# avik-pal/RegNeuralDE.jl

Hardware: AMD Instinct MI355X
Metric: training-step samples/sec + mean NFE, MNIST Neural ODE bs=512 (higher is better)
Workload: dtype f32; 1 GPU; MNIST NODE regularized (error_est), Tsit5 reltol=abstol=1.4e-8, batch 512 per GPU, 1xMI355X per rank; step = loss fwd + reverse pass through the solver + InvDecay/Momentum update; the weights train during the timed steps (mean_nfe drifts with --steps: value_fixed_weights of --full is the stationary companion); global_batch=512, parallelism=single

## Files before the change

regneuralde.jl_amd/csrc/rnde.hip:

```cpp
#include "rnde_node.h"

static thread_local std::string g_create_err;
extern "C" const char* rnde_version(void) { return "rnde 0.1.0 (gfx950)"; }
extern "C" const char* rnde_last_error(const rnde_node* h) { return h ? h->err.c_str() : g_create_err.c_str(); }

extern "C" int32_t rnde_param_count(const rnde_node_config* c) {
    int n = 0;
    for (int l = 0; l < c->n_layers; ++l) n += (c->dims[l] + (c->time_dep ? 1 : 0)) * c->dims[l + 1] + c->dims[l + 1];
    return n;
}

StepParams make_params(rnde_node* h, const float* x, int B, float t0, float t1, int tape) {
    StepParams P{};
    P.x = x;
    P.f0 = h->f0; P.h0 = h->h0; P.u1 = h->u1; P.f1 = h->f1; P.h1 = h->h1;
    P.arena = h->arena; P.rec_stride = h->rec_stride;
    P.ctl = h->ctl; P.ctl_final = h->ctl_final; P.meta = h->meta; P.initrec = h->initrec;
    P.errpart = h->errpart; P.initpart = h->initpart; P.dbg_out = nullptr;
    P.D = h->D; P.H = h->H; P.B = B; P.Bn = h->couple ? h->couple_batch : B;
    P.Bpad = ((B + 15) / 16) * 16;
    P.nwg = h->engine == 2 ? h->sR * (P.Bpad / 16) : (h->engine == 3 ? (h->mw ? P.Bpad / 16 : (P.Bpad / 16 + kCW - 1) / kCW) : P.Bpad / h->BT);
    P.reltol = h->cfg.reltol; P.abstol = h->cfg.abstol; P.t0 = t0; P.t1 = t1;
    P.tape = tape; P.max_attempts = h->cfg.max_attempts;
    P.forced = 0; P.forced_t = 0; P.forced_dt = 0;
// ... 513 lines not shown
    int n = 0;
    auto add = [&](void* dst, long long total, int kind, int which, int kdim, const float* src = nullptr) { J.j[n++] = PackJob{dst, src, total, kind, which, kdim, 0}; };
    add(h->spwB, (long long)h->sMT * h->sK2b * 64, 0, 0, h->sK2b);
    add(h->spwD, (long long)h->sHT * h->sMT * 64, 0, 1, h->sMT);
    add(h->spwBt, (long long)h->sMT * h->sKHb * 64, 0, 2, h->sKHb);
    add(h->spwDt, (long long)h->sHT * h->sMT * 64, 0, 3, h->sMT);
    auto add_copy = [&](float* dst, const float* src, long long floats) {
        const bool v4 = floats % 4 == 0 && ((uintptr_t)dst % 16 == 0) && ((uintptr_t)(src ? src : p_dev) % 16 == 0);
        add(dst, v4 ? floats / 4 : floats, v4 ? 3 : 2, 0, 0, src);
    };
    add_copy(h->pcopy, nullptr, (long long)h->P);
    if (x_src) add_copy(h->xcopy, x_src, x_floats);
    long long most = 0;
    for (int i = 0; i < n; ++i) most = std::max(most, J.j[i].total);
    const int grid = (int)std::min<long long>((most + 255) / 256, 256);
    hipLaunchKernelGGL(rnde_pack_all_kernel, dim3(grid, n), dim3(256), 0, s, p_dev, J, h->D, h->H);
    HIPCHK(h, hipGetLastError());
    h->rev_packed = true;
    return x3_pack(h, p_dev, true, s);
}
hipError_t slab_prepare(rnde_node* h, int Bpad, hipStream_t s) {
    if (h->tslab_Bpad == Bpad) return hipSuccess;
    h->tslab_Bpad = Bpad;
    return hipMemsetAsync(h->tslab, 0xFF, h->tslab_bytes, s);
}
static bool stage_two_tile(const rnde_node* h, const StageParams& Q) {
    const bool fix = Q.WT == 7 && Q.HT == 7 && Q.K2b == 7 && Q.MT == 49 && Q.R == 7 && h->D == 784 && h->H == 100 && !h->stage_generic;
    return h->persist == 1 && fix && Q.C % 2 == 0 && h->persist2 != 0 && (Q.C >= kPersist2MinTiles || h->persist2 >= 1);
}
static bool stage_epart_reduce(const rnde_node* h, const StageParams& Q) {
    return stage_two_tile(h, Q) && Q.F.nwg >= 896 && !getenv("RNDE_NO_EPART_REDUCE");
}
static hipError_t stage_attempt(rnde_node* h, const StageParams& Q, int n, hipStream_t s) {
// ... 231 lines not shown
            h->mw_solve = -1; h->mw_clean = 0; ++h->persist_fallbacks;
            hipMemsetAsync(h->mw_abort, 0, 8, s);
            return RNDE_INTERNAL_RETRY;
        }
        if (!h->h_ctl->done && h->h_ctl->n_att >= n_limit && n_limit < cap) { h->predicted = cap; return RNDE_INTERNAL_RETRY; }
        h->pending_bwd = false;
        ++h->one_launch_solves;
        solved = true;
    }
    if (h->engine == 2 && h->persist == 1 && h->stage_solve && h->sxch && SQ.C <= 32 && n_saveat == 0 && h->n_replay == 0 && !h->couple &&
        SQ.WT == 7 && SQ.HT == 7 && SQ.K2b == 7 && SQ.MT == 49 && SQ.R == 7 && h->D == 784 && h->H == 100 && !h->stage_generic) {
        PersistSync Y{h->tslab, h->pabort, h->pxcc, h->persist_spins};
        HIPCHK(h, slab_prepare(h, SQ.Bpad16, s));
        if (++h->s_epoch >= 500000u) { h->s_epoch = 1; HIPCHK(h, hipMemsetAsync(h->sxch, 0, (size_t)(cap + 1) * 3 * 256 * 8, s)); }
        const int x3 = h->x3_fwd ? 1 : 0;
        SolveSync Z{h->sxch, h->s_epoch, cap, h->x3B, h->x3D};
#ifdef RNDE_DIAG
        StageParams SD = SQ;
        if (getenv("RNDE_DIAG_SOLVE")) {
            if (h->diag_buf) hipFree(h->diag_buf);
            hipMalloc((void**)&h->diag_buf, 16384);
            hipMemsetAsync(h->diag_buf, 0, 16384, s);
            SD.F.dbg_out = h->diag_buf;
        }
        HIPCHK(h, rnde_launch_stage_solve(&SD, &Y, &Z, h->act2, x3, s));
#else
        HIPCHK(h, rnde_launch_stage_solve(&SQ, &Y, &Z, h->act2, x3, s));
#endif
        if (h->timing) { HIPCHK(h, hipEventRecord(h->tev[1], s)); h->tev_fwd = true; }
        hipLaunchKernelGGL(rnde_stage_finish_kernel, dim3(256), dim3(256), 0, s, SQ, -1, u_out_dev); HIPCHK(h, hipGetLastError());
        const int cnt = std::min(cap, std::max(64, 2 * h->predicted));
        HIPCHK(h, hipMemcpyAsync(h->h_mbox, h->mbox, h->mbox_meta_off + (size_t)cnt * sizeof(StepMeta), hipMemcpyDeviceToHost, s));
        if (h->after_solve) {
            HIPCHK(h, hipEventRecord(h->ev_host, s));
            const rnde_status hs = h->after_solve(s);
            if (hs != RNDE_OK) return hs;
            HIPCHK(h, hipEventSynchronize(h->ev_host));
        } else HIPCHK(h, hipStreamSynchronize(s));
#ifdef RNDE_DIAG
        if (getenv("RNDE_DIAG_SOLVE") && h->diag_buf) {
            static unsigned long long hst[1024];
            hipMemcpy(hst, h->diag_buf, 8192, hipMemcpyDeviceToHost);
            int na = 0; while (na < 119 && hst[(na + 1) * 8]) ++na;
            double acc[7] = {0}; int cnt = 0;
            for (int a = 2; a + 1 < na; ++a, ++cnt) {
// ... 431 lines not shown
```

regneuralde.jl_amd/csrc/rnde_bwd.h:

```cpp
#pragma once
#include "rnde_fwd.h"

namespace rnde {

struct BState {
    double tb_pre, dtb_pre, qoldb, t1b, t0b, pad[3];
};
struct IBState {
    double tb, t1b, t0b, dt0b, d1b, d2b, coef_w, pad;
};
struct EvalDesc {
    const float* Z;
    const float* X;
    float t;
    int pad;
};

struct BwdParams {
    StepParams F;
    float* U; float* K1; float* UB1;
    float* zi2; float* zi1;
    const float* svb_att;
    BState* bstate;
    IBState* ibstate;
// ... 79 lines not shown
static __global__ __launch_bounds__(64) void rnde_bpart_reduce_kernel(const BwdParams Q, int m, double* __restrict__ out) {
    const int lane = threadIdx.x;
    const float* part = Q.bpart + (size_t)(m & 1) * Q.bpart_n * 4;
    double S = 0, tau = 0, ctau = 0;
    for (int base = 0; base < Q.bpart_n; base += 256) {
        f32x4 e[4];
#pragma unroll
        for (int q = 0; q < 4; ++q) e[q] = *(const f32x4*)(part + 4 * (size_t)(base + lane + 64 * q));
#pragma unroll
        for (int q = 0; q < 4; ++q) if (base + lane + 64 * q < Q.bpart_n) { S += (double)e[q][0]; tau += (double)e[q][1]; ctau += (double)e[q][2]; }
    }
    S = wave_sum_d(S); tau = wave_sum_d(tau); ctau = wave_sum_d(ctau);
    if (lane == 0) { double* o = out + 4 * (m & 1); o[0] = S; o[1] = tau; o[2] = ctau; o[3] = 0; }
}

static __global__ __launch_bounds__(64) void rnde_bfin_kernel(const BwdParams Q) {
    const int lane = threadIdx.x;
    const IBState ib = Q.ibstate[1];
    double tau0 = 0;
    for (int i = lane; i < Q.F.nwg; i += 64) tau0 += (double)Q.ipart[((size_t)Q.F.nwg + i) * 4];
    tau0 = wave_sum_d(tau0);
    if (lane == 0) {
        const double sc = Q.tspan_scale != 0.f ? (double)Q.tspan_scale : 1.0;
        Q.tspan_out[0] = (float)(sc * (ib.t0b + tau0 + ib.tb));
        Q.tspan_out[1] = (float)(sc * ib.t1b);
    }
}

typedef float f32x16 __attribute__((ext_vector_type(16)));
__device__ __forceinline__ f32x4 mfma16(float a, float b, f32x4 c);

template <int MB, int NB>
__global__ __launch_bounds__(64) void rnde_wgrad_kernel(const EvalDesc* __restrict__ evals, int n_evals, int per_chunk,
                                                        int M, int Nx, int Bpad, float* __restrict__ slab) {
    const int lane = threadIdx.x, l31 = lane & 31, kk = lane >> 5;
    const int mtiles = (M + 31) / 32, ntiles = (Nx + 2 + 31) / 32;
    const int mblocks = (mtiles + MB - 1) / MB;
    const int mb = blockIdx.x % mblocks, nb = blockIdx.x / mblocks;
    const int chunk = blockIdx.y;
    const int e0 = chunk * per_chunk, e1 = min(n_evals, e0 + per_chunk);
    f32x16 acc[MB][NB];
#pragma unroll
// ... 274 lines not shown
        int c = c0;
        for (; c + 8 <= c1; c += 8) {
            float v[8];
#pragma unroll
            for (int j = 0; j < 8; ++j) v[j] = __builtin_nontemporal_load(slab + (size_t)(c + j) * len + i);
#pragma unroll
            for (int j = 0; j < 8; ++j) s += v[j];
        }
        for (; c < c1; ++c) s += __builtin_nontemporal_load(slab + (size_t)c * len + i);
        o[i] = s;
    }
}

struct ReduceJob { const float* slab; float* out; long long len; int n_chunks, per_group; };
struct ReducePair { ReduceJob j[2]; };
static __global__ void rnde_wgrad_reduce_pair(const ReducePair R) {
    const ReduceJob J = R.j[blockIdx.z];
    const int c0 = blockIdx.y * J.per_group, c1 = min(J.n_chunks, c0 + J.per_group);
    if (c0 >= c1) return;
    float* o = J.out + (size_t)blockIdx.y * J.len;
    for (long long i = blockIdx.x * (long long)blockDim.x + threadIdx.x; i < J.len; i += (long long)gridDim.x * blockDim.x) {
        float s = 0.f;
        int c = c0;
        for (; c + 8 <= c1; c += 8) {
            float v[8];
#pragma unroll
            for (int j = 0; j < 8; ++j) v[j] = __builtin_nontemporal_load(J.slab + (size_t)(c + j) * J.len + i);
#pragma unroll
            for (int j = 0; j < 8; ++j) s += v[j];
        }
        for (; c < c1; ++c) s += __builtin_nontemporal_load(J.slab + (size_t)c * J.len + i);
        o[i] = s;
    }
}

}
```

regneuralde.jl_amd/csrc/rnde_node.h:

```cpp
#pragma once
#include "../../include/rnde.h"
#include "rnde_fwd.h"
#include "rnde_bwd.h"
#include "rnde_stage.h"
#include "rnde_bstage.h"
#include "rnde_stage_persist2.h"
#include "rnde_bstage_persist.h"
#include "rnde_solve_sync.h"
#include "rnde_binit_stage.h"
#include "rnde_head.h"
#include "rnde_chain.h"
#include "rk_tables.h"
#include "rnde_bchain.h"
#include "rnde_chainmw.h"
#include "rnde_bchainmw.h"

#include <chrono>
#include <algorithm>
#include <atomic>
#include <cmath>
#include <cstdlib>
#include <cstdio>
#include <cstring>
#include <functional>
// ... 70 lines not shown
    int n_saveval = 0;
    int timing = 0; hipEvent_t tev[5] = {nullptr, nullptr, nullptr, nullptr, nullptr}; bool tev_fwd = false, tev_bwd = false;
    std::string err;
};

#define HIPCHK(h, call)                                                                              \
    do {                                                                                             \
        hipError_t e__ = (call);                                                                     \
        if (e__ != hipSuccess) {                                                                     \
            (h)->err = std::string(#call) + ": " + hipGetErrorString(e__);                           \
            return RNDE_ERR_HIP;                                                                     \
        }                                                                                            \
    } while (0)

static const rnde_status RNDE_INTERNAL_RETRY = static_cast<rnde_status>(100);
StepParams make_params(rnde_node* h, const float* x, int B, float t0, float t1, int tape);
MwParams make_mw_params(rnde_node* h, const StepParams& P);
ChainParams make_chain_params(rnde_node* h, const StepParams& P);
rnde_status couple_sum(rnde_node* h, float* partials, long long count, hipStream_t s);
hipError_t stage_pack(rnde_node* h, const float* p, f32x4* dst, int which, int MTrows, int Kb, hipStream_t st);
rnde_status stage_pack_all(rnde_node* h, const float* p_dev, hipStream_t s, const float* x_src = nullptr, long long x_floats = 0);
hipError_t slab_prepare(rnde_node* h, int Bpad, hipStream_t s);
void persist_check_enqueue(rnde_node* h, int grid, hipStream_t s);
bool persist_check_result(rnde_node* h, int C, int R, hipStream_t s);
bool bsweep_failed(rnde_node* h, hipStream_t s);
rnde_status forward_impl(rnde_node* h, const float* x_dev, const float* p_dev, int32_t B, float t0, float t1,
                         float* u_out_dev, const float* saveat_host, int32_t n_saveat, float* sv_out_dev,
                         int64_t* nfe_out, float* saveval_host, int32_t* n_saveval_out, int32_t keep_tape, void* stream);
```

regneuralde.jl_amd/csrc/rnde_reverse.hip:

```cpp
#include "rnde_node.h"
#include "rnde_wgradx.h"

static rnde_status chain_bwd_run(rnde_node* h, const float* u_bar_dev, const float* saveval_bar_host, float* x_bar_dev,
                                 float* p_bar_dev, float* tspan_bar_host, hipStream_t s, bool sync = true, float* tspan_bar_dev = nullptr);
static rnde_status bwd_run(rnde_node* h, const float* u_bar_dev, const float* saveval_bar_host, float* x_bar_dev,
                           float* p_bar_dev, float* tspan_bar_host, hipStream_t s, bool sync = true, float* tspan_bar_dev = nullptr);


extern "C" rnde_status rnde_node_backward_async(rnde_node* h, const float* u_bar_dev, const float* saveval_bar_host, float* x_bar_dev,
                                                float* p_bar_dev, float* tspan_bar_dev, void* stream) {
    if (!h) return RNDE_ERR_BAD_ARG;
    if (!h->have_tape) { h->err = "no recorded forward"; return RNDE_ERR_NO_TAPE; }
    if (h->engine == 3) return chain_bwd_run(h, u_bar_dev, saveval_bar_host, x_bar_dev, p_bar_dev, nullptr, (hipStream_t)stream, false, tspan_bar_dev);
    return bwd_run(h, u_bar_dev, saveval_bar_host, x_bar_dev, p_bar_dev, nullptr, (hipStream_t)stream, false, tspan_bar_dev);
}

extern "C" rnde_status rnde_node_backward(rnde_node* h, const float* u_bar_dev, const float* saveval_bar_host,
                                          float* x_bar_dev, float* p_bar_dev, float* tspan_bar_host, void* stream) {
    if (!h) return RNDE_ERR_BAD_ARG;
    if (!h->have_tape) { h->err = "no recorded forward"; return RNDE_ERR_NO_TAPE; }
    if (h->engine == 3) return chain_bwd_run(h, u_bar_dev, saveval_bar_host, x_bar_dev, p_bar_dev, tspan_bar_host, (hipStream_t)stream);
    return bwd_run(h, u_bar_dev, saveval_bar_host, x_bar_dev, p_bar_dev, tspan_bar_host, (hipStream_t)stream);
}
extern "C" rnde_status rnde_node_backward_host(rnde_node* h, const float* u_bar, const float* saveval_bar, float* x_bar,
// ... 138 lines not shown
        if ((size_t)(*chunk_cursor + sc) * (size_t)len > h->bw.slab_floats) { h->err = "weight-gradient slab overflow"; return RNDE_ERR_BAD_ARG; }
        if (tall) hipLaunchKernelGGL((rnde_wgrad2_kernel<true>), dim3(pblocks, sc), dim3(256), 0, s, ev, n_evals, steps_per_chunk, M, Nx, Bpad, dst);
        else hipLaunchKernelGGL((rnde_wgrad2_kernel<false>), dim3(pblocks, sc), dim3(256), 0, s, ev, n_evals, steps_per_chunk, M, Nx, Bpad, dst);
        HIPCHK(h, hipGetLastError());
        *chunk_cursor += sc;
        return RNDE_OK;
    } else {
        if ((size_t)(*chunk_cursor + chunks) * (size_t)len > h->bw.slab_floats) { h->err = "weight-gradient slab overflow"; return RNDE_ERR_BAD_ARG; }
        if (tall) hipLaunchKernelGGL((rnde_wgrad_kernel<2, 4>), dim3(blocks, chunks), dim3(64), 0, s, ev, n_evals, per_chunk, M, Nx, Bpad, dst);
        else hipLaunchKernelGGL((rnde_wgrad_kernel<4, 2>), dim3(blocks, chunks), dim3(64), 0, s, ev, n_evals, per_chunk, M, Nx, Bpad, dst);
    }
    HIPCHK(h, hipGetLastError());
    *chunk_cursor += chunks;
    return RNDE_OK;
}
static rnde_status launch_wgrad_reduce(rnde_node* h, const float* slab, int chunks, int M, int Nx, float* out, hipStream_t s) {
    const long long len = (long long)M * (Nx + 2);
    const int grid = (int)std::min<long long>((len + 255) / 256, 2048);
    if (chunks <= 16) {
        hipLaunchKernelGGL(rnde_wgrad_reduce, dim3(grid, 1), dim3(256), 0, s, slab, chunks, chunks, len, out);
    } else {
        const int per_group = (chunks + 15) / 16, groups = (chunks + per_group - 1) / per_group;
        hipLaunchKernelGGL(rnde_wgrad_reduce, dim3(grid, groups), dim3(256), 0, s, slab, chunks, per_group, len, h->bw.slab_r);
        hipLaunchKernelGGL(rnde_wgrad_reduce, dim3(grid, 1), dim3(256), 0, s, (const float*)h->bw.slab_r, groups, groups, len, out);
    }
    HIPCHK(h, hipGetLastError());
    return RNDE_OK;
}

static rnde_status bwd_run(rnde_node* h, const float* u_bar_dev, const float* saveval_bar_host, float* x_bar_dev,
                           float* p_bar_dev, float* tspan_bar_host, hipStream_t s, bool sync, float* tspan_bar_dev) {
    HIPCHK(h, hipSetDevice(h->cfg.device));
    rnde_status st = bwd_prepare(h);
    if (st != RNDE_OK) return st;
    BwdBuffers& b = h->bw;
    int n_att = h->n_att;
    const float svb_scale = h->couple ? (float)h->couple_world : 1.f;
    for (int i = 0; i < n_att; ++i)
        b.h_svb[i] = (saveval_bar_host && h->sv_index[i] >= 0) ? svb_scale * saveval_bar_host[h->sv_index[i]] : 0.f;
// ... 23 lines not shown
    for (int n = 0; n < n_att; ++n) {
        const StepMeta& m = h->h_meta[n];
        const float* R = h->arena + (long long)m.rec * h->rec_stride;
        for (int sidx = 2; sidx <= 7; ++sidx) {
            const float ts = m.t + tsC(sidx - 1) * m.dt;
            h_ev2[ne] = EvalDesc{R + L.k(sidx), R + L.h(sidx), ts, 0};
            h_ev1[ne] = EvalDesc{R + L.z1(sidx), sidx < 7 ? R + L.g(sidx) : R + L.unew(), ts, 0};
            ++ne;
        }
    }
    HIPCHK(h, hipMemcpyAsync(b.ev1, b.h_ev1, 2 * (size_t)ne * sizeof(EvalDesc) + (size_t)n_att * 4, hipMemcpyHostToDevice, s));
    float* slab1 = b.slab;
    float* slab2w = b.slab + b.slab_floats;
    int cur1 = 0, cur2 = 0, evi = 0;
    const int per_chunk = std::max(1, (ne + 239) / 240);
    const int side_pct = h->wgrad_side_pct;
    const int sweep_cus = 8 * h->sR * ((Q.F.Bpad / 16 + 7) / 8);
    const bool side = h->engine == 2 && h->persist == 1 && side_pct > 0 && n_att >= 8 && sweep_cus <= 224 &&
                      wgrad3_ok(h->H, h->D) && wgrad3_ok(h->D, h->H);
    const int side_att = side ? std::min(n_att, n_att * side_pct / 100) : 0;
    const int group = std::max(4, (side_att + 5) / 6);
    bool used_side = false;
    auto wgrad_group = [&](int lo, int hi, bool on_side) -> rnde_status {
        if (hi <= lo) return RNDE_OK;
        hipStream_t ws = s;
        if (on_side) {
            hipEvent_t ev = h->wevents[evi++ % 64];
            HIPCHK(h, hipEventRecord(ev, s));
            HIPCHK(h, hipStreamWaitEvent(h->wstream, ev, 0));
            ws = h->wstream; used_side = true;
        }
        rnde_status r = launch_wgrad_part(h, d_ev1 + lo, hi - lo, per_chunk, h->H, h->D, h->B, slab1, &cur1, ws, on_side ? 16 : 0);
        if (r != RNDE_OK) return r;
        return launch_wgrad_part(h, d_ev2 + lo, hi - lo, per_chunk, h->D, h->H, h->B, slab2w, &cur2, ws, on_side ? 16 : 0);
    };
    int hi_att = n_att;
    hipError_t e;
    h->tev_bwd = false;
    if (h->timing) HIPCHK(h, hipEventRecord(h->tev[2], s));
    if (h->engine == 2) {
        if (!h->rev_packed) {
            HIPCHK(h, stage_pack(h, h->pcopy, h->spwBt, 2, h->sMT, h->sKHb, s));
            HIPCHK(h, stage_pack(h, h->pcopy, h->spwDt, 3, h->sHT, h->sMT, s));
        }
        h->rev_packed = false;
// ... 91 lines not shown
                hipLaunchKernelGGL((rnde_binit_stage_kernel<1, 0>), grid, blk, h->stage_lds, s, BQ);
                hipLaunchKernelGGL((rnde_binit_stage_kernel<1, 1>), grid, blk, h->stage_lds, s, BQ);
            } else {
                hipLaunchKernelGGL((rnde_binit_stage_kernel<0, 0>), grid, blk, h->stage_lds, s, BQ);
                hipLaunchKernelGGL((rnde_binit_stage_kernel<0, 1>), grid, blk, h->stage_lds, s, BQ);
            }
            if ((st = couple_sum(h, Q.ipart, 4LL * Q.F.nwg, s)) != RNDE_OK) return st;
            if (h->act2) {
                hipLaunchKernelGGL((rnde_binit_stage_kernel<1, 2>), grid, blk, h->stage_lds, s, BQ);
                hipLaunchKernelGGL((rnde_binit_stage_kernel<1, 3>), grid, blk, h->stage_lds, s, BQ);
            } else {
                hipLaunchKernelGGL((rnde_binit_stage_kernel<0, 2>), grid, blk, h->stage_lds, s, BQ);
                hipLaunchKernelGGL((rnde_binit_stage_kernel<0, 3>), grid, blk, h->stage_lds, s, BQ);
            }
            if ((st = couple_sum(h, Q.ipart + 4LL * Q.F.nwg, 4LL * Q.F.nwg, s)) != RNDE_OK) return st;
            hipLaunchKernelGGL(rnde_bfin_kernel, dim3(1), dim3(64), 0, s, Q);
            HIPCHK(h, hipGetLastError());
        }
    }
    if (h->timing) HIPCHK(h, hipEventRecord(h->tev[3], s));
    st = wgrad_group(0, 2 + 6 * hi_att, false);
    if (st != RNDE_OK) return st;
    if (used_side) {
        hipEvent_t ev = h->wevents[64];
        HIPCHK(h, hipEventRecord(ev, h->wstream));
        HIPCHK(h, hipStreamWaitEvent(s, ev, 0));
    }
    if (cur1 > 16 && cur2 > 16) {
        const long long len1 = (long long)h->H * (h->D + 2), len2 = (long long)h->D * (h->H + 2);
        const size_t seg_r = std::max((size_t)len1, (size_t)len2);
        float* r1 = b.slab_r; float* r2 = b.slab_r + 16 * seg_r;
        const int pg1 = (cur1 + 15) / 16, g1 = (cur1 + pg1 - 1) / pg1, pg2 = (cur2 + 15) / 16, g2 = (cur2 + pg2 - 1) / pg2;
        const int grid = (int)std::min<long long>((std::max(len1, len2) + 255) / 256, 2048);
        ReducePair A{{{slab1, r1, len1, cur1, pg1}, {slab2w, r2, len2, cur2, pg2}}};
        hipLaunchKernelGGL(rnde_wgrad_reduce_pair, dim3(grid, std::max(g1, g2), 2), dim3(256), 0, s, A);
        ReducePair Bp{{{r1, p_bar_dev, len1, g1, g1}, {r2, p_bar_dev + (size_t)h->H * (h->D + 2), len2, g2, g2}}};
        hipLaunchKernelGGL(rnde_wgrad_reduce_pair, dim3(grid, 1, 2), dim3(256), 0, s, Bp);
        HIPCHK(h, hipGetLastError());
    } else {
        st = launch_wgrad_reduce(h, slab1, cur1, h->H, h->D, p_bar_dev, s);
        if (st != RNDE_OK) return st;
        st = launch_wgrad_reduce(h, slab2w, cur2, h->D, h->H, p_bar_dev + (size_t)h->H * (h->D + 2), s);
        if (st != RNDE_OK) return st;
    }
    if (h->timing) { HIPCHK(h, hipEventRecord(h->tev[4], s)); h->tev_bwd = true; }
#ifdef RNDE_DIAG
    if (h->engine == 2 && h->persist == 1 && getenv("RNDE_DIAG_BWD")) {
        unsigned long long hst[64] = {0};
        hipStreamSynchronize(s);
        hipMemcpy(hst, h->diag_buf, sizeof(hst), hipMemcpyDeviceToHost);
        fprintf(stderr, "persistent reverse attempt (workgroup 0 thread 0, cycles): START %lld (entry->weights issued %lld, ->w1t %lld, ->array loads issued %lld, finish_attempt_scalars %lld, scalar chain %lld, vector part %lld), its phase D + put %lld\n", (long long)(hst[1]-hst[0]), (long long)(hst[43]-hst[0]), (long long)(hst[44]-hst[43]), (long long)(hst[40]-hst[44]), (long long)(hst[41]-hst[40]), (long long)(hst[42]-hst[41]), (long long)(hst[1]-hst[42]), (long long)(hst[2]-hst[1]));
        for (int st = 0; st < 6; ++st) { const unsigned long long* q = hst + 3 + 5 * st; const unsigned long long prev = st == 0 ? hst[2] : hst[7 + 5 * (st - 1)];
            fprintf(stderr, "  stage j=%d: poll %lld A %lld B %lld C %lld D+put %lld\n", 6 - st, (long long)(q[0]-prev), (long long)(q[1]-q[0]), (long long)(q[2]-q[1]), (long long)(q[3]-q[2]), st < 5 ? (long long)(q[4]-q[3]) : 0LL); }
        fprintf(stderr, "  total %lld cycles to the end of stage 1, END (reduction of the 21 partial sums) %lld; in START's vector part the wait for the record's k arrays %lld\n",
                (long long)(hst[34]-hst[0]), (long long)(hst[35]-hst[34]), (long long)(hst[45]-hst[42]));
    }
#endif
// ... 417 lines not shown
```

regneuralde.jl_amd/csrc/rnde_solve_sync.h:

```cpp
#pragma once

namespace rnde {

struct SolveSync {
    unsigned long long* xch;
    unsigned epoch;
    int n_limit;
    const void* x3B;
    const void* x3D;
};

}
```

regneuralde.jl_amd/csrc/rnde_stage.h:

```cpp
#pragma once
#include "rnde_fwd.h"

namespace rnde {

constexpr int kSCB = 16;
constexpr int kSMaxW = 8;
constexpr int kSMaxHT = 8;

struct StageParams {
    StepParams F;
    const float* p;
    const f32x4* pwB;
    const f32x4* pwD;
    float* slab;
    int MT, WT, R, C, HT, K2b;
    int Bpad16;
};

__device__ __forceinline__ int kperm(int k) { return (k & ~15) | ((k & 3) << 2) | ((k >> 2) & 3); }

__device__ __forceinline__ f32x4 mfma16(float a, float b, f32x4 c) {
    return __builtin_amdgcn_mfma_f32_16x16x4f32(a, b, c, 0, 0, 0);
}
__device__ __forceinline__ float add_square_unfused(float acc, float d) {
// ... 22 lines not shown
        else if (which == 2) { if (m < D && k < H) w = W1[(size_t)m * H + k]; }
        else { if (m <= H && k < D) w = W2[(size_t)m * D + k]; }
        v[q] = w;
    }
    return v;
}
static __global__ void rnde_stage_pack_kernel(const float* __restrict__ p, f32x4* __restrict__ dst, int which, int D, int H,
                                       int MTrows, int Kb) {
    const long long total = (long long)MTrows * Kb * 64;
    for (long long i = blockIdx.x * (long long)blockDim.x + threadIdx.x; i < total; i += (long long)gridDim.x * blockDim.x)
        dst[i] = stage_pack_elem(p, which, D, H, Kb, i);
}

struct PackJob { void* dst; const float* src; long long total; int kind, which, kdim, pad; };
struct PackJobs { PackJob j[8]; };
static __global__ void rnde_pack_all_kernel(const float* __restrict__ p, const PackJobs J, int D, int H) {
    const PackJob job = J.j[blockIdx.y];
    for (long long i = blockIdx.x * (long long)blockDim.x + threadIdx.x; i < job.total; i += (long long)gridDim.x * blockDim.x) {
        if (job.kind == 0) ((f32x4*)job.dst)[i] = stage_pack_elem(p, job.which, D, H, job.kdim, i);
        else if (job.kind == 2) ((float*)job.dst)[i] = (job.src ? job.src : p)[i];
        else ((f32x4*)job.dst)[i] = ((const f32x4*)(job.src ? job.src : p))[i];
    }
}

__device__ __forceinline__ void dense_points(const StepParams& P, const RecLayout& L, const float* Rp, float tp, float dtp_, float tnew,
                                             int lo, int hi, size_t co, int gcol, int r0, bool colok, bool vec) {
    const f32x4 up = ld_tile(Rp + L.upc() + co, r0, P.D, true, vec);
    f32x4 k[7];
    k[0] = ld_tile(Rp + L.k1c() + co, r0, P.D, true, vec);
#pragma unroll
    for (int j = 1; j < 7; ++j) k[j] = ld_tile(Rp + L.k(j + 1) + co, r0, P.D, true, vec);
    const f32x4 un = ld_tile(Rp + L.unew() + co, r0, P.D, true, vec);
    for (int idx = lo; idx < hi; ++idx) {
        const float ts = P.sv_t[idx];
        f32x4 o = un;
        if (ts != tnew) {
            float b[7];
// ... 407 lines not shown
```

regneuralde.jl_amd/csrc/rnde_stage_solve.h:

```cpp
#pragma once
#ifndef RNDE_SOLVE_DEFER_TAPE
#define RNDE_SOLVE_DEFER_TAPE 1
#endif
#ifndef RNDE_SOLVE_LOCAL_LAYOUT
#define RNDE_SOLVE_LOCAL_LAYOUT 1
#endif
#include "rnde_stage_persist.h"
#include "rnde_solve_sync.h"
#include "rnde_x3.h"

namespace rnde {

typedef __attribute__((address_space(1))) unsigned long long solve_gu64;

__device__ __forceinline__ bool solve_meet(const SolveSync& Z, const PersistSync& Y, int seq, int nwg, int wg, int nval, const float (&mine)[3],
                                           double (&out)[3], int lane) {
    const unsigned tag = Z.epoch * 8192u + (unsigned)seq + 1u;
    solve_gu64* base = (solve_gu64*)Z.xch + (size_t)seq * 3 * 256;
    if (lane == 0) {
#pragma unroll
        for (int v = 0; v < 3; ++v) {
            if (v < nval) {
                float m = mine[v];
                if (m != m) m = __uint_as_float(0x7FC00000u);
// ... 166 lines not shown
    StepState S{};
    if (w == 0) {
        const StepState nop{};
        S = advance_state_t<true>(P, 0, lane, writer, &P.ctl[0], none, nop, nullptr, nullptr);
        if (lane == 0) solve_state_put(SS, S);
    }
    __syncthreads();
    S = solve_state_get(SS);
    f32x4 c_un = {0.f, 0.f, 0.f, 0.f};
    constexpr bool DEFER = RNDE_SOLVE_DEFER_TAPE && X3;
    f32x4 pend = {0.f, 0.f, 0.f, 0.f};
    for (int n = 0;; ++n) {
        ZSTAMP(0);
        if (w == 3 && lane == 0) QP[(n + 1) & 1] = powf(S.qold, P.beta2);
        ZSTAMP(1);
        if (S.done || n >= Z.n_limit) { if (writer) *P.ctl_final = S; return; }
        const float t = S.t, dt = (P.t1 - S.t < S.dtp) ? (P.t1 - S.t) : S.dtp;
        const int rec = P.tape ? n : (S.live == 0 ? 1 : 0);
        float* R = P.arena + (long long)rec * P.rec_stride;
#if RNDE_SOLVE_LOCAL_LAYOUT
        long long A_n = LL.A, HB_n = LL.HB;
        asm volatile("" : "+s"(A_n), "+s"(HB_n));
        const RecLayout L{A_n, HB_n};
#endif

        {
            const f32x4 v = fma4(dt, tsA(1, 0) * c_k[0], c_up);
            slab_clears_done();
            if constexpr (DEFER) pend = v;
            else if (P.tape) st4(R + L.g(2) + co, r0, gD, true, vec, v);
            phase_d(v, 1u);
// ... 150 lines not shown
```

regneuralde.jl_amd/csrc/rnde_wgradx.h:

```cpp
#pragma once
#include "rnde_x3.h"

namespace rnde {

constexpr int kWxRowShorts = 40;
constexpr int kWxTallRows = 400, kWxNarrowRows = 112;
constexpr int kWxPlaneShortsT = kWxTallRows * kWxRowShorts, kWxPlaneShortsS = kWxNarrowRows * kWxRowShorts;
constexpr size_t kWxLdsBytes = (size_t)3 * (kWxPlaneShortsT + kWxPlaneShortsS) * 2;

template <bool TALL_IS_Z>
__global__ __launch_bounds__(448) void rnde_wgrad3x_kernel(const EvalDesc* __restrict__ evals, int n_evals, int per_chunk, int M, int Nx, int Bpad, float* __restrict__ slab) {
    constexpr int KC = 32;
    extern __shared__ __attribute__((aligned(16))) unsigned short wxs[];
    unsigned short* TP = wxs;
    unsigned short* SP = wxs + 3 * kWxPlaneShortsT;
    const int tid = threadIdx.x, lane = tid & 63, w = __builtin_amdgcn_readfirstlane(tid >> 6);
    const int mrow = lane & 15, kk = lane >> 4;
    const int TR = TALL_IS_Z ? M : Nx + 2, SR = TALL_IS_Z ? Nx + 2 : M;
    const int TRp = TALL_IS_Z ? M : Nx, SRp = TALL_IS_Z ? Nx : M;
    const int TT = (TR + 15) >> 4, T0 = (TT + 1) >> 1;
    const int half = blockIdx.x, chunk = blockIdx.y;
    const int tile_lo = half ? T0 : 0, tile_hi = half ? TT : T0, ntile = tile_hi - tile_lo;
    const int row_lo = 16 * tile_lo, nrow = 16 * ntile;
    const int steps_per_eval = (Bpad + KC - 1) / KC;
// ... 118 lines not shown
#ifndef RNDE_WX4_ABL
#define RNDE_WX4_ABL 0
#endif
constexpr int kWx4TallRows = 208;
constexpr int kWx4PlaneT = kWx4TallRows * kWxRowShorts, kWx4PlaneS = kWxNarrowRows * kWxRowShorts;
constexpr int kWx4ImageShorts = 3 * (kWx4PlaneT + kWx4PlaneS);
constexpr size_t kWx4LdsBytes = (size_t)2 * kWx4ImageShorts * 2;
constexpr int kWx4fRowShorts = 32;
constexpr int kWx4fWideShorts = (kWx4TallRows + 4) * kWx4fRowShorts;
constexpr int kWx4fPlane = (kWx4TallRows + 4 + kWxNarrowRows + 4) * kWx4fRowShorts;
constexpr int kWx4fImageShorts = 3 * kWx4fPlane;
constexpr size_t kWx4fLdsBytes = (size_t)2 * kWx4fImageShorts * 2;
constexpr int kWx4DefaultFeed = 1;

template <bool TALL_IS_Z, int FEED>
__global__ __launch_bounds__(448) void rnde_wgrad4x_kernel(const EvalDesc* __restrict__ evals, int n_evals, int per_chunk, int n_chunks, int M, int Nx, int Bpad,
                                                           float* __restrict__ slab) {
    constexpr int KC = 32;
    extern __shared__ __attribute__((aligned(16))) unsigned short wxs[];
    const int tid = threadIdx.x, lane = tid & 63, w = __builtin_amdgcn_readfirstlane(tid >> 6);
    const int mrow = lane & 15, kk = lane >> 4;
    const int lin = blockIdx.x, xcd = lin & 7, within = lin >> 3;
    const int chunk = (within >> 2) * 8 + xcd, part = within & 3;
    if (chunk >= n_chunks) return;
    const int TR = TALL_IS_Z ? M : Nx + 2, SR = TALL_IS_Z ? Nx + 2 : M;
    const int TRp = TALL_IS_Z ? M : Nx, SRp = TALL_IS_Z ? Nx : M;
    const int TT = (TR + 15) >> 4, base = TT >> 2, rem = TT & 3;
    const int ntile = base + (part < rem ? 1 : 0), tile_lo = part * base + (part < rem ? part : rem);
    const int row_lo = 16 * tile_lo, nrow = 16 * ntile;
    const int steps_per_eval = (Bpad + KC - 1) / KC;
    const int s_lo = chunk * per_chunk, s_hi = min(n_evals * steps_per_eval, s_lo + per_chunk);
    const int total_steps = max(0, s_hi - s_lo);
    x3f4 acc[2][7];
#pragma unroll
    for (int i = 0; i < 2; ++i)
#pragma unroll
        for (int n = 0; n < 7; ++n) acc[i][n] = (x3f4){0.f, 0.f, 0.f, 0.f};
// ... 151 lines not shown
#pragma unroll
    for (int i = 0; i < 2; ++i) {
        if (w + 7 * i < ntile) {
#pragma unroll
            for (int n = 0; n < 7; ++n) {
                const int sr = 16 * n + mrow;
#pragma unroll
                for (int q = 0; q < 4; ++q) {
                    const int tr = row_lo + 16 * (w + 7 * i) + 4 * kk + q;
                    if (tr < TR && sr < SR) out[TALL_IS_Z ? (size_t)sr * M + tr : (size_t)tr * M + sr] = acc[i][n][q];
                }
            }
        }
    }
}

}
```

regneuralde.jl_amd/csrc/rnde_x3.h:

```cpp
#pragma once
#include <hip/hip_runtime.h>

namespace rnde {

typedef unsigned x3u4 __attribute__((ext_vector_type(4)));
typedef unsigned x3u2 __attribute__((ext_vector_type(2)));
typedef __bf16 x3bf8 __attribute__((ext_vector_type(8)));
typedef float x3f4 __attribute__((ext_vector_type(4)));

constexpr int kX3K = 136;
constexpr int kX3PlaneShorts = 16 * kX3K;
constexpr int kX3ImageFloats = 3 * kX3PlaneShorts / 2;

__device__ __forceinline__ unsigned x3_cvt2(float a, float b) {
    unsigned r;
    asm("v_cvt_pk_bf16_f32 %0, %1, %2" : "=v"(r) : "v"(a), "v"(b));
    return r;
}
#ifndef RNDE_X3_DOT2
#define RNDE_X3_DOT2 0
#endif
typedef __bf16 x3bf2 __attribute__((ext_vector_type(2)));
typedef float x3f2 __attribute__((ext_vector_type(2)));
__device__ __forceinline__ void x3_split2(float x0, float x1, unsigned& hi, unsigned& mid, unsigned& lo) {
// ... 43 lines not shown
        if (s + 1 < NS) { nh = x3_frag(img, 0, s + 1, lane); nm = x3_frag(img, 1, s + 1, lane); nl = x3_frag(img, 2, s + 1, lane); }
        __builtin_amdgcn_sched_barrier(0);
        aL = x3_mfma(wa[s][2], bh, aL);
        aM = x3_mfma(wa[s][1], bh, aM);
        aH = x3_mfma(wa[s][0], bh, aH);
        aN = x3_mfma(wa[s][1], bm, aN);
        aL = x3_mfma(wa[s][0], bl, aL);
        aM = x3_mfma(wa[s][0], bm, aM);
        __builtin_amdgcn_sched_barrier(0);
        bh = nh; bm = nm; bl = nl;
    }
    return ((aL + aN) + aM) + aH;
}

struct X3PackDst { x3u4* d[4]; };
static __global__ void rnde_x3_pack_kernel(const float* __restrict__ p, const X3PackDst dst, int D, int H, int MT, int WT, int R, int HT) {
    const float* W1 = p;
    const float* b1 = W1 + (size_t)H * (D + 1);
    const float* W2 = b1 + H;
    const float* b2 = W2 + (size_t)D * (H + 1);
    const long long nB = (long long)MT * 4 * 64, nD = (long long)HT * R * 4 * 64, per = nB + nD;
    const int nimg = dst.d[2] ? 2 : 1;
    for (long long i = blockIdx.x * (long long)blockDim.x + threadIdx.x; i < nimg * per; i += (long long)gridDim.x * blockDim.x) {
        const int rev = (int)(i / per);
        const long long ii = i - rev * per;
        const bool isD = ii >= nB;
        const long long q = isD ? ii - nB : ii;
        const int l = (int)(q & 63), s = (int)((q >> 6) & 3), tile = (int)(q >> 8);
        float wv[8];
#pragma unroll
        for (int j = 0; j < 8; ++j) {
            const int k = 32 * s + 8 * (l >> 4) + j;
            float w = 0.f;
            if (!isD) {
                const int m = 16 * tile + (l & 15);
                if (m < D) {
                    if (!rev) w = k <= H ? W2[(size_t)k * D + m] : (k == H + 1 ? b2[m] : 0.f);
                    else if (k < H) w = W1[(size_t)m * H + k];
// ... 5 lines not shown
                    if (!rev) { if (m < H) w = W1[(size_t)row * H + m]; }
                    else if (m <= H) w = W2[(size_t)m * D + row];
                }
            }
            wv[j] = w;
        }
        unsigned hi[4], mid[4], lo[4];
#pragma unroll
        for (int j = 0; j < 4; ++j) x3_split2(wv[2 * j], wv[2 * j + 1], hi[j], mid[j], lo[j]);
        x3u4* o = dst.d[2 * rev + (isD ? 1 : 0)] + ((size_t)(tile * 4 + s) * 3) * 64 + l;
        o[0] = (x3u4){hi[0], hi[1], hi[2], hi[3]};
        o[64] = (x3u4){mid[0], mid[1], mid[2], mid[3]};
        o[128] = (x3u4){lo[0], lo[1], lo[2], lo[3]};
    }
}

}
```

Before: 310,700 samples/s.

## Fold small launches into neighbouring kernels to cut per-step launch count

Adds a RNDE_LAUNCH_DIET bitmask, enabled by default, that merges several small kernels into their neighbours. The x3 weight pack joins the general pack kernel as an extra grid row. The persistent solve kernel writes u_out itself instead of using a separate finish kernel. The backward-finish wave rides as an extra block of the last weight-gradient reduce, and the two weight-gradient layers run in one tail kernel. The aim is to remove kernel launch and dependency gaps per training step, at the cost of more branching in the kernels and some extra blocks that can sit idle.

```diff
diff --git a/regneuralde.jl_amd/csrc/rnde.hip b/regneuralde.jl_amd/csrc/rnde.hip
--- a/regneuralde.jl_amd/csrc/rnde.hip
+++ b/regneuralde.jl_amd/csrc/rnde.hip
@@ -551,9 +551,18 @@
     long long most = 0;
     for (int i = 0; i < n; ++i) most = std::max(most, J.j[i].total);
     const int grid = (int)std::min<long long>((most + 255) / 256, 256);
+    h->rev_packed = true;
+    if ((launch_diet() & kDietPacks) && h->x3 && h->x3B && h->x3D && h->persist == 1 && !h->stage_generic) {
+        const bool rev = h->x3Bt && h->x3Dt;
+        const X3PackDst xd{{(x3u4*)h->x3B, (x3u4*)h->x3D, rev ? (x3u4*)h->x3Bt : nullptr, rev ? (x3u4*)h->x3Dt : nullptr}};
+        hipLaunchKernelGGL(rnde_pack_all_x3_kernel, dim3(grid, n + 1), dim3(256), 0, s, p_dev, J, n, h->D, h->H, xd, h->sMT, h->sWT, h->sR, h->sHT);
+        HIPCHK(h, hipGetLastError());
+        h->x3_fwd = true;
+        h->x3_packed = true;
+        return RNDE_OK;
+    }
     hipLaunchKernelGGL(rnde_pack_all_kernel, dim3(grid, n), dim3(256), 0, s, p_dev, J, h->D, h->H);
     HIPCHK(h, hipGetLastError());
-    h->rev_packed = true;
     return x3_pack(h, p_dev, true, s);
 }
 hipError_t slab_prepare(rnde_node* h, int Bpad, hipStream_t s) {
@@ -815,7 +824,8 @@
         HIPCHK(h, slab_prepare(h, SQ.Bpad16, s));
         if (++h->s_epoch >= 500000u) { h->s_epoch = 1; HIPCHK(h, hipMemsetAsync(h->sxch, 0, (size_t)(cap + 1) * 3 * 256 * 8, s)); }
         const int x3 = h->x3_fwd ? 1 : 0;
-        SolveSync Z{h->sxch, h->s_epoch, cap, h->x3B, h->x3D};
+        const bool own_u_out = u_out_dev && (launch_diet() & kDietFinish) != 0;
+        SolveSync Z{h->sxch, h->s_epoch, cap, h->x3B, h->x3D, own_u_out ? u_out_dev : nullptr, ((uintptr_t)u_out_dev % 16 == 0) ? 1 : 0};
 #ifdef RNDE_DIAG
         StageParams SD = SQ;
         if (getenv("RNDE_DIAG_SOLVE")) {
@@ -829,7 +839,7 @@
         HIPCHK(h, rnde_launch_stage_solve(&SQ, &Y, &Z, h->act2, x3, s));
 #endif
         if (h->timing) { HIPCHK(h, hipEventRecord(h->tev[1], s)); h->tev_fwd = true; }
-        hipLaunchKernelGGL(rnde_stage_finish_kernel, dim3(256), dim3(256), 0, s, SQ, -1, u_out_dev); HIPCHK(h, hipGetLastError());
+        if (!own_u_out) { hipLaunchKernelGGL(rnde_stage_finish_kernel, dim3(256), dim3(256), 0, s, SQ, -1, u_out_dev); HIPCHK(h, hipGetLastError()); }
         const int cnt = std::min(cap, std::max(64, 2 * h->predicted));
         HIPCHK(h, hipMemcpyAsync(h->h_mbox, h->mbox, h->mbox_meta_off + (size_t)cnt * sizeof(StepMeta), hipMemcpyDeviceToHost, s));
         if (h->after_solve) {
diff --git a/regneuralde.jl_amd/csrc/rnde_bwd.h b/regneuralde.jl_amd/csrc/rnde_bwd.h
--- a/regneuralde.jl_amd/csrc/rnde_bwd.h
+++ b/regneuralde.jl_amd/csrc/rnde_bwd.h
@@ -117,8 +117,7 @@
     if (lane == 0) { double* o = out + 4 * (m & 1); o[0] = S; o[1] = tau; o[2] = ctau; o[3] = 0; }
 }
 
-static __global__ __launch_bounds__(64) void rnde_bfin_kernel(const BwdParams Q) {
-    const int lane = threadIdx.x;
+__device__ __forceinline__ void bfin_wave(const BwdParams& Q, const int lane) {
     const IBState ib = Q.ibstate[1];
     double tau0 = 0;
     for (int i = lane; i < Q.F.nwg; i += 64) tau0 += (double)Q.ipart[((size_t)Q.F.nwg + i) * 4];
@@ -129,6 +128,7 @@
         Q.tspan_out[1] = (float)(sc * ib.t1b);
     }
 }
+static __global__ __launch_bounds__(64) void rnde_bfin_kernel(const BwdParams Q) { bfin_wave(Q, threadIdx.x); }
 
 typedef float f32x16 __attribute__((ext_vector_type(16)));
 __device__ __forceinline__ f32x4 mfma16(float a, float b, f32x4 c);
@@ -433,12 +433,11 @@
 
 struct ReduceJob { const float* slab; float* out; long long len; int n_chunks, per_group; };
 struct ReducePair { ReduceJob j[2]; };
-static __global__ void rnde_wgrad_reduce_pair(const ReducePair R) {
-    const ReduceJob J = R.j[blockIdx.z];
-    const int c0 = blockIdx.y * J.per_group, c1 = min(J.n_chunks, c0 + J.per_group);
+__device__ __forceinline__ void wgrad_reduce_job(const ReduceJob& J, const int bx, const int gx, const int by) {
+    const int c0 = by * J.per_group, c1 = min(J.n_chunks, c0 + J.per_group);
     if (c0 >= c1) return;
-    float* o = J.out + (size_t)blockIdx.y * J.len;
-    for (long long i = blockIdx.x * (long long)blockDim.x + threadIdx.x; i < J.len; i += (long long)gridDim.x * blockDim.x) {
+    float* o = J.out + (size_t)by * J.len;
+    for (long long i = bx * (long long)blockDim.x + threadIdx.x; i < J.len; i += (long long)gx * blockDim.x) {
         float s = 0.f;
         int c = c0;
         for (; c + 8 <= c1; c += 8) {
@@ -452,5 +451,13 @@
         o[i] = s;
     }
 }
-
-}
+static __global__ void rnde_wgrad_reduce_pair(const ReducePair R) { wgrad_reduce_job(R.j[blockIdx.z], (int)blockIdx.x, (int)gridDim.x, (int)blockIdx.y); }
+static __global__ void rnde_wgrad_reduce_pair_fin(const ReducePair R, const BwdParams Q) {
+    if (blockIdx.x + 1 == gridDim.x) {
+        if (blockIdx.y == 0 && blockIdx.z == 0 && threadIdx.x < 64) bfin_wave(Q, (int)threadIdx.x);
+        return;
+    }
+    wgrad_reduce_job(R.j[blockIdx.z], (int)blockIdx.x, (int)gridDim.x - 1, (int)blockIdx.y);
+}
+
+}
diff --git a/regneuralde.jl_amd/csrc/rnde_node.h b/regneuralde.jl_amd/csrc/rnde_node.h
--- a/regneuralde.jl_amd/csrc/rnde_node.h
+++ b/regneuralde.jl_amd/csrc/rnde_node.h
@@ -108,6 +108,11 @@
     } while (0)
 
 static const rnde_status RNDE_INTERNAL_RETRY = static_cast<rnde_status>(100);
+enum : unsigned { kDietFinish = 4u, kDietBfin = 8u, kDietTailGemm = 16u, kDietPacks = 32u };
+static inline unsigned launch_diet() {
+    const char* e = getenv("RNDE_LAUNCH_DIET");
+    return e ? (unsigned)strtoul(e, nullptr, 0) : ~0u;
+}
 StepParams make_params(rnde_node* h, const float* x, int B, float t0, float t1, int tape);
 MwParams make_mw_params(rnde_node* h, const StepParams& P);
 ChainParams make_chain_params(rnde_node* h, const StepParams& P);
diff --git a/regneuralde.jl_amd/csrc/rnde_reverse.hip b/regneuralde.jl_amd/csrc/rnde_reverse.hip
--- a/regneuralde.jl_amd/csrc/rnde_reverse.hip
+++ b/regneuralde.jl_amd/csrc/rnde_reverse.hip
@@ -176,15 +176,60 @@
     *chunk_cursor += chunks;
     return RNDE_OK;
 }
-static rnde_status launch_wgrad_reduce(rnde_node* h, const float* slab, int chunks, int M, int Nx, float* out, hipStream_t s) {
+static rnde_status launch_wgrad_tail_pair(rnde_node* h, const EvalDesc* ev1, const EvalDesc* ev2, int n_evals, int Bpad, float* slab1, int* cur1,
+                                          float* slab2, int* cur2, hipStream_t s, bool& launched) {
+    launched = false;
+#if RNDE_WX4_ABL == 7 || RNDE_WX4_ABL == 8
+    return RNDE_OK;
+#else
+    const int H = h->H, D = h->D;
+    const int TT1 = (D + 2 + 15) / 16, TT2 = (D + 15) / 16;
+    if (n_evals <= 0 || !wgrad3_ok(H, D) || !wgrad3_ok(D, H) || H >= D || !h->x3_packed || getenv("RNDE_X3_WGRAD_OFF") || getenv("RNDE_X3_WGRAD_HALF") ||
+        TT1 < 28 || TT1 > 52 || TT2 < 28 || TT2 > 52) return RNDE_OK;
+    const int total_steps = n_evals * ((Bpad + 31) / 32);
+    static const int target_chunks = getenv("RNDE_WGRAD3_CHUNKS") ? atoi(getenv("RNDE_WGRAD3_CHUNKS")) : 128;
+    static const int target4 = getenv("RNDE_WGRAD4_CHUNKS") ? atoi(getenv("RNDE_WGRAD4_CHUNKS")) : 64;
+    int sc = std::max(1, std::min({target_chunks, total_steps, 256}));
+    const int steps_per_chunk = (total_steps + sc - 1) / sc;
+    sc = (total_steps + steps_per_chunk - 1) / steps_per_chunk;
+    int sc4 = std::max(1, std::min({target4, total_steps, 256}));
+    const int spc4 = (total_steps + sc4 - 1) / sc4;
+    sc4 = (total_steps + spc4 - 1) / spc4;
+    const size_t len1 = (size_t)H * (D + 2), len2 = (size_t)D * (H + 2);
+    if ((size_t)(*cur1 + std::max(sc, sc4)) * len1 > h->bw.slab_floats || (size_t)(*cur2 + std::max(sc, sc4)) * len2 > h->bw.slab_floats) {
+        h->err = "weight-gradient slab overflow"; return RNDE_ERR_BAD_ARG;
+    }
+    static DeviceOnce attrt;
+    if (attrt.need()) {
+        HIPCHK(h, hipFuncSetAttribute((const void*)rnde_wgrad4x_tail_kernel<0>, hipFuncAttributeMaxDynamicSharedMemorySize, (int)kWx4LdsBytes));
+        HIPCHK(h, hipFuncSetAttribute((const void*)rnde_wgrad4x_tail_kernel<1>, hipFuncAttributeMaxDynamicSharedMemorySize, (int)kWx4fLdsBytes));
+        attrt.done();
+    }
+    const int g1 = 32 * ((sc4 + 7) / 8);
+    const Wx4Layer l1{ev1, slab1 + (size_t)(*cur1) * len1, spc4, sc4, H, D}, l2{ev2, slab2 + (size_t)(*cur2) * len2, spc4, sc4, D, H};
+    const char* ef = getenv("RNDE_X3_WGRAD_FEED");
+    const bool q0 = getenv("RNDE_X3_WGRAD_Q0") != nullptr || (ef ? ef[0] == '0' : kWx4DefaultFeed == 0);
+    if (q0) hipLaunchKernelGGL((rnde_wgrad4x_tail_kernel<0>), dim3(2 * g1), dim3(448), kWx4LdsBytes, s, l1, l2, g1, n_evals, Bpad);
+    else hipLaunchKernelGGL((rnde_wgrad4x_tail_kernel<1>), dim3(2 * g1), dim3(448), kWx4fLdsBytes, s, l1, l2, g1, n_evals, Bpad);
+    HIPCHK(h, hipGetLastError());
+    *cur1 += sc4; *cur2 += sc4;
+    launched = true;
+    return RNDE_OK;
+#endif
+}
+static rnde_status launch_wgrad_reduce(rnde_node* h, const float* slab, int chunks, int M, int Nx, float* out, hipStream_t s, const BwdParams* fin = nullptr) {
     const long long len = (long long)M * (Nx + 2);
     const int grid = (int)std::min<long long>((len + 255) / 256, 2048);
+    auto last = [&](const float* src, int n) {
+        if (fin) hipLaunchKernelGGL(rnde_wgrad_reduce_pair_fin, dim3(grid + 1, 1, 1), dim3(256), 0, s, ReducePair{{{src, out, len, n, n}, {}}}, *fin);
+        else hipLaunchKernelGGL(rnde_wgrad_reduce, dim3(grid, 1), dim3(256), 0, s, src, n, n, len, out);
+    };
     if (chunks <= 16) {
-        hipLaunchKernelGGL(rnde_wgrad_reduce, dim3(grid, 1), dim3(256), 0, s, slab, chunks, chunks, len, out);
+        last(slab, chunks);
     } else {
         const int per_group = (chunks + 15) / 16, groups = (chunks + per_group - 1) / per_group;
         hipLaunchKernelGGL(rnde_wgrad_reduce, dim3(grid, groups), dim3(256), 0, s, slab, chunks, per_group, len, h->bw.slab_r);
-        hipLaunchKernelGGL(rnde_wgrad_reduce, dim3(grid, 1), dim3(256), 0, s, (const float*)h->bw.slab_r, groups, groups, len, out);
+        last((const float*)h->bw.slab_r, groups);
     }
     HIPCHK(h, hipGetLastError());
     return RNDE_OK;
@@ -238,6 +283,8 @@
     float* slab2w = b.slab + b.slab_floats;
     int cur1 = 0, cur2 = 0, evi = 0;
     const int per_chunk = std::max(1, (ne + 239) / 240);
+    const unsigned diet = launch_diet();
+    const bool fold_bfin = h->engine == 2 && (diet & kDietBfin) != 0;
     const int side_pct = h->wgrad_side_pct;
     const int sweep_cus = 8 * h->sR * ((Q.F.Bpad / 16 + 7) / 8);
     const bool side = h->engine == 2 && h->persist == 1 && side_pct > 0 && n_att >= 8 && sweep_cus <= 224 &&
@@ -253,6 +300,10 @@
             HIPCHK(h, hipEventRecord(ev, s));
             HIPCHK(h, hipStreamWaitEvent(h->wstream, ev, 0));
             ws = h->wstream; used_side = true;
+        } else if (diet & kDietTailGemm) {
+            bool launched = false;
+            rnde_status r = launch_wgrad_tail_pair(h, d_ev1 + lo, d_ev2 + lo, hi - lo, h->B, slab1, &cur1, slab2w, &cur2, ws, launched);
+            if (r != RNDE_OK || launched) return r;
         }
         rnde_status r = launch_wgrad_part(h, d_ev1 + lo, hi - lo, per_chunk, h->H, h->D, h->B, slab1, &cur1, ws, on_side ? 16 : 0);
         if (r != RNDE_OK) return r;
@@ -374,7 +425,7 @@
                 hipLaunchKernelGGL((rnde_binit_stage_kernel<0, 3>), grid, blk, h->stage_lds, s, BQ);
             }
             if ((st = couple_sum(h, Q.ipart + 4LL * Q.F.nwg, 4LL * Q.F.nwg, s)) != RNDE_OK) return st;
-            hipLaunchKernelGGL(rnde_bfin_kernel, dim3(1), dim3(64), 0, s, Q);
+            if (!fold_bfin) hipLaunchKernelGGL(rnde_bfin_kernel, dim3(1), dim3(64), 0, s, Q);
             HIPCHK(h, hipGetLastError());
         }
     }
@@ -395,12 +446,13 @@
         ReducePair A{{{slab1, r1, len1, cur1, pg1}, {slab2w, r2, len2, cur2, pg2}}};
         hipLaunchKernelGGL(rnde_wgrad_reduce_pair, dim3(grid, std::max(g1, g2), 2), dim3(256), 0, s, A);
         ReducePair Bp{{{r1, p_bar_dev, len1, g1, g1}, {r2, p_bar_dev + (size_t)h->H * (h->D + 2), len2, g2, g2}}};
-        hipLaunchKernelGGL(rnde_wgrad_reduce_pair, dim3(grid, 1, 2), dim3(256), 0, s, Bp);
+        if (fold_bfin) hipLaunchKernelGGL(rnde_wgrad_reduce_pair_fin, dim3(grid + 1, 1, 2), dim3(256), 0, s, Bp, Q);
+        else hipLaunchKernelGGL(rnde_wgrad_reduce_pair, dim3(grid, 1, 2), dim3(256), 0, s, Bp);
         HIPCHK(h, hipGetLastError());
     } else {
         st = launch_wgrad_reduce(h, slab1, cur1, h->H, h->D, p_bar_dev, s);
         if (st != RNDE_OK) return st;
-        st = launch_wgrad_reduce(h, slab2w, cur2, h->D, h->H, p_bar_dev + (size_t)h->H * (h->D + 2), s);
+        st = launch_wgrad_reduce(h, slab2w, cur2, h->D, h->H, p_bar_dev + (size_t)h->H * (h->D + 2), s, fold_bfin ? &Q : nullptr);
         if (st != RNDE_OK) return st;
     }
     if (h->timing) { HIPCHK(h, hipEventRecord(h->tev[4], s)); h->tev_bwd = true; }
diff --git a/regneuralde.jl_amd/csrc/rnde_solve_sync.h b/regneuralde.jl_amd/csrc/rnde_solve_sync.h
--- a/regneuralde.jl_amd/csrc/rnde_solve_sync.h
+++ b/regneuralde.jl_amd/csrc/rnde_solve_sync.h
@@ -8,6 +8,8 @@
     int n_limit;
     const void* x3B;
     const void* x3D;
+    float* u_out;
+    int u_vec;
 };
 
 }
diff --git a/regneuralde.jl_amd/csrc/rnde_stage.h b/regneuralde.jl_amd/csrc/rnde_stage.h
--- a/regneuralde.jl_amd/csrc/rnde_stage.h
+++ b/regneuralde.jl_amd/csrc/rnde_stage.h
@@ -1,5 +1,6 @@
 #pragma once
 #include "rnde_fwd.h"
+#include "rnde_x3.h"
 
 namespace rnde {
 
@@ -60,13 +61,21 @@
 
 struct PackJob { void* dst; const float* src; long long total; int kind, which, kdim, pad; };
 struct PackJobs { PackJob j[8]; };
-static __global__ void rnde_pack_all_kernel(const float* __restrict__ p, const PackJobs J, int D, int H) {
-    const PackJob job = J.j[blockIdx.y];
+__device__ __forceinline__ void pack_job_items(const float* __restrict__ p, const PackJob& job, int D, int H) {
     for (long long i = blockIdx.x * (long long)blockDim.x + threadIdx.x; i < job.total; i += (long long)gridDim.x * blockDim.x) {
         if (job.kind == 0) ((f32x4*)job.dst)[i] = stage_pack_elem(p, job.which, D, H, job.kdim, i);
         else if (job.kind == 2) ((float*)job.dst)[i] = (job.src ? job.src : p)[i];
         else ((f32x4*)job.dst)[i] = ((const f32x4*)(job.src ? job.src : p))[i];
     }
+}
+static __global__ void rnde_pack_all_kernel(const float* __restrict__ p, const PackJobs J, int D, int H) { pack_job_items(p, J.j[blockIdx.y], D, H); }
+static __global__ void rnde_pack_all_x3_kernel(const float* __restrict__ p, const PackJobs J, const int njobs, int D, int H, const X3PackDst x3, int MT, int WT,
+                                               int R, int HT) {
+    if ((int)blockIdx.y == njobs) {
+        x3_pack_items(p, x3, D, H, MT, WT, R, HT, blockIdx.x * (long long)blockDim.x + threadIdx.x, (long long)gridDim.x * blockDim.x);
+        return;
+    }
+    pack_job_items(p, J.j[blockIdx.y], D, H);
 }
 
 __device__ __forceinline__ void dense_points(const StepParams& P, const RecLayout& L, const float* Rp, float tp, float dtp_, float tnew,
diff --git a/regneuralde.jl_amd/csrc/rnde_stage_solve.h b/regneuralde.jl_amd/csrc/rnde_stage_solve.h
--- a/regneuralde.jl_amd/csrc/rnde_stage_solve.h
+++ b/regneuralde.jl_amd/csrc/rnde_stage_solve.h
@@ -204,7 +204,11 @@
         ZSTAMP(0);
         if (w == 3 && lane == 0) QP[(n + 1) & 1] = powf(S.qold, P.beta2);
         ZSTAMP(1);
-        if (S.done || n >= Z.n_limit) { if (writer) *P.ctl_final = S; return; }
+        if (S.done || n >= Z.n_limit) {
+            if (writer) *P.ctl_final = S;
+            if (Z.u_out) st4(Z.u_out + co, r0, gD, colok, Z.u_vec != 0, c_up);
+            return;
+        }
         const float t = S.t, dt = (P.t1 - S.t < S.dtp) ? (P.t1 - S.t) : S.dtp;
         const int rec = P.tape ? n : (S.live == 0 ? 1 : 0);
         float* R = P.arena + (long long)rec * P.rec_stride;
diff --git a/regneuralde.jl_amd/csrc/rnde_wgradx.h b/regneuralde.jl_amd/csrc/rnde_wgradx.h
--- a/regneuralde.jl_amd/csrc/rnde_wgradx.h
+++ b/regneuralde.jl_amd/csrc/rnde_wgradx.h
@@ -156,13 +156,13 @@
 constexpr int kWx4DefaultFeed = 1;
 
 template <bool TALL_IS_Z, int FEED>
-__global__ __launch_bounds__(448) void rnde_wgrad4x_kernel(const EvalDesc* __restrict__ evals, int n_evals, int per_chunk, int n_chunks, int M, int Nx, int Bpad,
-                                                           float* __restrict__ slab) {
+__device__ __forceinline__ void wgrad4x_body(const int lin, const EvalDesc* __restrict__ evals, int n_evals, int per_chunk, int n_chunks, int M, int Nx, int Bpad,
+                                             float* __restrict__ slab) {
     constexpr int KC = 32;
     extern __shared__ __attribute__((aligned(16))) unsigned short wxs[];
     const int tid = threadIdx.x, lane = tid & 63, w = __builtin_amdgcn_readfirstlane(tid >> 6);
     const int mrow = lane & 15, kk = lane >> 4;
-    const int lin = blockIdx.x, xcd = lin & 7, within = lin >> 3;
+    const int xcd = lin & 7, within = lin >> 3;
     const int chunk = (within >> 2) * 8 + xcd, part = within & 3;
     if (chunk >= n_chunks) return;
     const int TR = TALL_IS_Z ? M : Nx + 2, SR = TALL_IS_Z ? Nx + 2 : M;
@@ -344,5 +344,18 @@
         }
     }
 }
-
-}
+template <bool TALL_IS_Z, int FEED>
+__global__ __launch_bounds__(448) void rnde_wgrad4x_kernel(const EvalDesc* __restrict__ evals, int n_evals, int per_chunk, int n_chunks, int M, int Nx, int Bpad,
+                                                           float* __restrict__ slab) {
+    wgrad4x_body<TALL_IS_Z, FEED>((int)blockIdx.x, evals, n_evals, per_chunk, n_chunks, M, Nx, Bpad, slab);
+}
+
+struct Wx4Layer { const EvalDesc* evals; float* slab; int per_chunk, n_chunks, M, Nx; };
+template <int FEED>
+__global__ __launch_bounds__(448) void rnde_wgrad4x_tail_kernel(const Wx4Layer l1, const Wx4Layer l2, int g1, int n_evals, int Bpad) {
+    const int lin = (int)blockIdx.x;
+    if (lin < g1) wgrad4x_body<false, FEED>(lin, l1.evals, n_evals, l1.per_chunk, l1.n_chunks, l1.M, l1.Nx, Bpad, l1.slab);
+    else wgrad4x_body<true, FEED>(lin - g1, l2.evals, n_evals, l2.per_chunk, l2.n_chunks, l2.M, l2.Nx, Bpad, l2.slab);
+}
+
+}
diff --git a/regneuralde.jl_amd/csrc/rnde_x3.h b/regneuralde.jl_amd/csrc/rnde_x3.h
--- a/regneuralde.jl_amd/csrc/rnde_x3.h
+++ b/regneuralde.jl_amd/csrc/rnde_x3.h
@@ -81,14 +81,15 @@
 }
 
 struct X3PackDst { x3u4* d[4]; };
-static __global__ void rnde_x3_pack_kernel(const float* __restrict__ p, const X3PackDst dst, int D, int H, int MT, int WT, int R, int HT) {
+__device__ __forceinline__ void x3_pack_items(const float* __restrict__ p, const X3PackDst& dst, int D, int H, int MT, int WT, int R, int HT, const long long first,
+                                              const long long stride) {
     const float* W1 = p;
     const float* b1 = W1 + (size_t)H * (D + 1);
     const float* W2 = b1 + H;
     const float* b2 = W2 + (size_t)D * (H + 1);
     const long long nB = (long long)MT * 4 * 64, nD = (long long)HT * R * 4 * 64, per = nB + nD;
     const int nimg = dst.d[2] ? 2 : 1;
-    for (long long i = blockIdx.x * (long long)blockDim.x + threadIdx.x; i < nimg * per; i += (long long)gridDim.x * blockDim.x) {
+    for (long long i = first; i < nimg * per; i += stride) {
         const int rev = (int)(i / per);
         const long long ii = i - rev * per;
         const bool isD = ii >= nB;
@@ -124,5 +125,8 @@
         o[128] = (x3u4){lo[0], lo[1], lo[2], lo[3]};
     }
 }
+static __global__ void rnde_x3_pack_kernel(const float* __restrict__ p, const X3PackDst dst, int D, int H, int MT, int WT, int R, int HT) {
+    x3_pack_items(p, dst, D, H, MT, WT, R, HT, blockIdx.x * (long long)blockDim.x + threadIdx.x, (long long)gridDim.x * blockDim.x);
+}
 
 }
```

After: 313,000 samples/s, median of 6. No clear change (+0.7%).
